# GeoStat-Framework/PyKrige

Hardware: NVIDIA H100
Metric: kriged grid points/sec (N data -> M grid) (higher is better)
Workload: dtype f64

## Files before the change

pykrige_b200/csrc/api.cu:

```cuda
#include <cuda_runtime.h>
#include <string>
#include <vector>
#include <cstring>
#include <cstdio>
#include <cmath>
#include <cstdlib>
#include <algorithm>
#include <thread>
#include <climits>
#include "kernels.h"

#define KB_VERSION 2000
static const int64_t KB_STAGE_PTS = 1 << 20;
#define KB_TILE_COST_32 0.607
#define KB_TILE_COST_16 0.403
static const int64_t KB_STAGE_MIN = 1 << 18;
#define KB_TN_FIELDS 32

struct Src {
    bool grid; int64_t nx, ny, nz;
    const double *a, *b, *c;
    int64_t first, count;
    const double* d_drift; int64_t drift_stride, drift_first;
};

#define KB_GJ_DEFAULT_BLOCKED 1

struct DevBuf {
    void* p = nullptr; size_t cap = 0;
    cudaError_t reserve(size_t bytes) {
        if (bytes <= cap) return cudaSuccess;
        if (p) cudaFree(p);
        p = nullptr; cap = 0;
        cudaError_t e = cudaMalloc(&p, bytes);
        if (e == cudaSuccess) cap = bytes;
        return e;
    }
    void release() { if (p) cudaFree(p); p = nullptr; cap = 0; }
    template <typename T> T* as() const { return reinterpret_cast<T*>(p); }
};

struct kb200_ctx {
    int device = 0;
    cudaStream_t stream = nullptr;
    bool own_stream = false;
    std::string err;

    bool described = false, ready = false, knn_ready = false;
    bool factor_live = false;
    bool inv_live = false;
    int slices = 0;
    int gform = 0;
    int geo = 0;
    int pinv = 0;
    int pinv_sweeps = 0, pinv_rank = 0;
    int dim = 2, dtype = KB200_F64, n = 0, n_pad = 0, ld = 0, n_rl = 0, n_hd = 0, K1 = 1, na = 2, nrb = 0;
    VgParams vg{};
    Aniso an{};
    DriftScale ds{};
    PackMap pm{};
    std::vector<double> hx, hy, hz, hval, hdrift;
    double bb_lo[3] = {0, 0, 0}, bb_hi[3] = {0, 0, 0};
    int nf = 0; int64_t nf_n = 0;
    std::vector<double> hfields;
    int aux_cols = KB_MAXAUX;
    int64_t zstride = 0;
    int pin_blocks = 0;

    DevBuf blob;
    size_t off_consts = 0, off_ax = 0, off_ay = 0, off_az = 0, off_tiles = 0, off_rowscale = 0, blob_bytes = 0;

    DevBuf wC, wW, wT, wF, wRaw, wFlag;
    DevBuf wPart, wAux, wPts, wOut, wAxes, wDrift, wScratch, wFstage;
    int num_sms = 132;
    DeviceDrift dd{};
    DevBuf wWells, wExt;
    int n_dev = 0;
    void* pin[2] = {nullptr, nullptr};
    cudaStream_t copy_stream = nullptr;
    cudaEvent_t evk[2] = {}, evc[2] = {};
    cudaStream_t hi_stream = nullptr;
    std::vector<cudaEvent_t> fev;
    DevBuf kSorted, kCells, kFields;
    DevBuf wVario;
    DevBuf wLoo;
    DevBuf wTab;
    std::vector<double> htab;
    double tab_dmax = 0.0; int tab_n = 0;
    KnnParams kp{};
    int k_ncells = 0;

    cudaEvent_t ev[16] = {};
    double tm[12] = {};
    long long launches = 0, solve_launches = 0;
};

static int fail(kb200_ctx* h, int code, const std::string& msg) {
    if (h) h->err = msg;
    return code;
}
#define CU(h, expr) do { cudaError_t _e = (expr); if (_e != cudaSuccess) { \
    return fail(h, _e == cudaErrorMemoryAllocation ? KB200_ENOMEM : KB200_ECUDA, \
                std::string(#expr) + ": " + cudaGetErrorString(_e)); } } while (0)

static size_t align_up(size_t v, size_t a) { return (v + a - 1) / a * a; }

extern "C" int kb200_version(void) { return KB_VERSION; }

extern "C" int kb200_create(kb200_handle* out, int device) {
    if (!out) return KB200_EBADARG;
    *out = nullptr;
    int cnt = 0;
    cudaError_t e = cudaGetDeviceCount(&cnt);
    if (e != cudaSuccess || cnt == 0) return KB200_ECUDA;
    kb200_ctx* h = new kb200_ctx();
    if (device < 0) { if (cudaGetDevice(&device) != cudaSuccess) device = 0; }
    if (device >= cnt) { delete h; return KB200_EBADARG; }
    h->device = device;
    if (cudaSetDevice(device) != cudaSuccess) { delete h; return KB200_ECUDA; }
    if (cudaStreamCreateWithFlags(&h->stream, cudaStreamNonBlocking) != cudaSuccess) { delete h; return KB200_ECUDA; }
    h->own_stream = true;
    for (auto& ev : h->ev) if (cudaEventCreate(&ev) != cudaSuccess) { delete h; return KB200_ECUDA; }
    if (kbk_factor_init() != cudaSuccess || kbk_solve_init() != cudaSuccess || kbk_solve_tf32_init() != cudaSuccess ||
        kbk_solve_i8_init() != cudaSuccess || kbk_ev_init() != cudaSuccess || kbk_pinv_init() != cudaSuccess) { delete h; return KB200_ECUDA; }
    if (cudaDeviceGetAttribute(&h->num_sms, cudaDevAttrMultiProcessorCount, device) != cudaSuccess || h->num_sms < 1) h->num_sms = 132;
    *out = h;
    return KB200_OK;
}

extern "C" void kb200_destroy(kb200_handle h) {
    if (!h) return;
    cudaSetDevice(h->device);
    cudaStreamSynchronize(h->stream);
    for (DevBuf* b : {&h->blob, &h->wC, &h->wW, &h->wT, &h->wF, &h->wRaw, &h->wFlag, &h->wPart, &h->wAux,
                      &h->wPts, &h->wOut, &h->wAxes, &h->wDrift, &h->wScratch, &h->wFstage, &h->kSorted, &h->kCells, &h->kFields, &h->wVario, &h->wTab,
                      &h->wLoo, &h->wWells, &h->wExt}) b->release();
    for (int i = 0; i < 2; ++i) {
        if (h->pin[i]) cudaFreeHost(h->pin[i]);
        if (h->evk[i]) cudaEventDestroy(h->evk[i]);
        if (h->evc[i]) cudaEventDestroy(h->evc[i]);
    }
    if (h->copy_stream) cudaStreamDestroy(h->copy_stream);
    if (h->hi_stream) cudaStreamDestroy(h->hi_stream);
    for (auto& e : h->fev) cudaEventDestroy(e);
    for (auto& ev : h->ev) if (ev) cudaEventDestroy(ev);
    if (h->own_stream && h->stream) cudaStreamDestroy(h->stream);
    delete h;
}

extern "C" const char* kb200_last_error(kb200_handle h) { return h ? h->err.c_str() : "null handle"; }

extern "C" int kb200_set_stream(kb200_handle h, void* s) {
    if (!h) return KB200_EBADARG;
    if (h->own_stream && h->stream) { cudaStreamSynchronize(h->stream); cudaStreamDestroy(h->stream); }
    h->stream = reinterpret_cast<cudaStream_t>(s);
    h->own_stream = false;
    return KB200_OK;
}

extern "C" int kb200_set_coordinates(kb200_handle h, int coordinates_type) {
    if (!h) return KB200_EBADARG;
    if (coordinates_type != KB200_EUCLIDEAN && coordinates_type != KB200_GEOGRAPHIC)
        return fail(h, KB200_EBADARG, "coordinates_type must be KB200_EUCLIDEAN or KB200_GEOGRAPHIC");
    h->geo = coordinates_type == KB200_GEOGRAPHIC ? 1 : 0;
    h->described = false; h->ready = false; h->knn_ready = false; h->factor_live = false;
    return KB200_OK;
}

extern "C" int kb200_set_pseudo_inverse(kb200_handle h, int enable) {
    if (!h) return KB200_EBADARG;
    h->pinv = enable ? 1 : 0;
    h->described = false; h->ready = false; h->knn_ready = false; h->factor_live = false;
    return KB200_OK;
}

extern "C" int kb200_set_values(kb200_handle h, int n_fields, int64_t n, const double* values) {
    if (!h) return KB200_EBADARG;
    h->described = false; h->ready = false; h->knn_ready = false; h->factor_live = false;
    h->nf = 0; h->nf_n = 0; h->hfields.clear();
    if (n_fields == 0) return KB200_OK;
    if (n_fields < 0 || n_fields > KB200_MAX_FIELDS)
        return fail(h, KB200_EBADARG, "n_fields must be in [0, " + std::to_string(KB200_MAX_FIELDS) + "]");
    if (n < 1 || n > (1LL << 30) || !values) return fail(h, KB200_EBADARG, "values: n >= 1 rows and a non-NULL array");
    const size_t cnt = (size_t)n * n_fields;
    for (size_t i = 0; i < cnt; ++i)
        if (!std::isfinite(values[i]))
            return fail(h, KB200_EBADARG, "values must be finite (field " + std::to_string(i / n) + ", row " +
                        std::to_string(i % n) + ")");
    h->hfields.assign(values, values + cnt);
    h->nf = n_fields; h->nf_n = n;
    return KB200_OK;
}

extern "C" void kb200_reset_counters(kb200_handle h) {
    if (!h) return;
    h->launches = 0; h->solve_launches = 0;
    for (double& t : h->tm) t = 0.0;
}

extern "C" int kb200_last_timings(kb200_handle h, double* ms, int n) {
    if (!h || !ms) return KB200_EBADARG;
    h->tm[10] = (double)h->solve_launches;
    h->tm[11] = (double)h->launches;
    int m = std::min(n, 12);
    for (int i = 0; i < m; ++i) ms[i] = h->tm[i];
    return m;
// ... 348 lines not shown
    CU(h, kbk_dual(h->wW.as<double>(), ld, nn, np, h->n_rl, h->n_hd, nv, ax, ay, az, h->ds, rh, vals,
                   Fz, Hz, Uz, consts, flag, st, &launches));
    if (h->dtype == KB200_F32) {
        CU(h, kbk_pack_tf32(h->wW.as<double>(), ld, nn, np, h->na, Uz, h->pm, blob + h->off_tiles, st));
    } else if (h->slices) {
        const int nrb8 = kbk_i8_nrb(h->slices, nn, h->na);
        std::vector<long long> toff(nrb8 + 1);
        kbk_i8_total_tiles(h->slices, nn, h->na, toff.data());
        long long* d_toff = reinterpret_cast<long long*>(h->wT.as<char>());
        int* d_rowexp = reinterpret_cast<int*>(h->wT.as<char>() + align_up((size_t)(nrb8 + 1) * sizeof(long long), 256));
        CU(h, cudaMemcpyAsync(d_toff, toff.data(), (size_t)(nrb8 + 1) * sizeof(long long), cudaMemcpyHostToDevice, st));
        CU(h, kbk_pack_i8(h->slices, h->wW.as<double>(), ld, nn, np, h->na, Uz, d_rowexp,
                          reinterpret_cast<double*>(blob + h->off_rowscale), d_toff, blob + h->off_tiles, st));
        CU(h, cudaStreamSynchronize(st));
        ++launches;
    } else {
        CU(h, kbk_pack(h->dtype, h->wW.as<double>(), ld, nn, np, h->na, Uz, h->pm, blob + h->off_tiles, st));
    }
    ++launches;
    }
    double hdr[64] = {0};
    hdr[0] = KB_MAGIC; hdr[1] = h->vg.c0; hdr[34] = (double)h->gform;
    for (int c = 0; c <= KB200_MAX_DRIFT; ++c) { hdr[2 + c] = h->ds.shift[c]; hdr[18 + c] = h->ds.scale[c]; }
    CU(h, cudaMemcpyAsync(blob, hdr, sizeof(hdr), cudaMemcpyHostToDevice, st));
    CU(h, cudaEventRecord(h->ev[6], st));
    CU(h, cudaMemcpyAsync(&hflag, flag, sizeof(int), cudaMemcpyDeviceToHost, st));
    CU(h, cudaStreamSynchronize(st));
    h->tm[6] += ev_ms(h->ev[0], h->ev[1]);
    h->tm[0] += t_asm; h->tm[1] += t_chol;
    h->tm[2] += ev_ms(h->ev[4], h->ev[5]);
    h->tm[3] += ev_ms(h->ev[5], h->ev[6]);
    h->launches += launches;
    if (hflag != 0) return fail(h, KB200_ESINGULAR, "drift/unbiasedness block F^T C^-1 F is singular");
    h->ready = true;
    h->factor_live = !h->gform;
    h->inv_live = h->gform != 2;
    return KB200_OK;
}

extern "C" int kb200_set_device_drift(kb200_handle h, int n_wells, const double* wells,
                                      int64_t ext_nx, int64_t ext_ny, const double* ext_x, const double* ext_y,
                                      const double* ext_z) {
    if (!h) return KB200_EBADARG;
    if (n_wells < 0 || n_wells > KB200_MAX_DRIFT || (n_wells > 0 && !wells))
        return fail(h, KB200_EBADARG, "device drift: bad point_log description");
    const bool ext = ext_nx > 0 || ext_ny > 0;
    if (ext && (ext_nx < 1 || ext_ny < 1 || ext_nx > (1 << 30) || ext_ny > (1 << 30) || !ext_x || !ext_y || !ext_z))
        return fail(h, KB200_EBADARG, "device drift: bad external_Z raster description");
    h->described = false; h->ready = false; h->factor_live = false;
    cudaSetDevice(h->device);
    h->dd = DeviceDrift{};
    if (n_wells) {
        CU(h, h->wWells.reserve((size_t)3 * n_wells * 8));
        CU(h, cudaMemcpyAsync(h->wWells.p, wells, (size_t)3 * n_wells * 8, cudaMemcpyHostToDevice, h->stream));
        h->dd.n_wells = n_wells; h->dd.wells = h->wWells.as<double>();
    }
    if (ext) {
        const size_t nx = (size_t)ext_nx, ny = (size_t)ext_ny;
        CU(h, h->wExt.reserve((nx + ny + nx * ny) * 8));
        double* d = h->wExt.as<double>();
        CU(h, cudaMemcpyAsync(d, ext_x, nx * 8, cudaMemcpyHostToDevice, h->stream));
        CU(h, cudaMemcpyAsync(d + nx, ext_y, ny * 8, cudaMemcpyHostToDevice, h->stream));
        CU(h, cudaMemcpyAsync(d + nx + ny, ext_z, nx * ny * 8, cudaMemcpyHostToDevice, h->stream));
        bool sorted = true;
        for (size_t i = 1; i < nx && sorted; ++i) sorted = ext_x[i] >= ext_x[i - 1];
        for (size_t i = 1; i < ny && sorted; ++i) sorted = ext_y[i] >= ext_y[i - 1];
        h->dd.ext = 1; h->dd.ext_nx = (int)ext_nx; h->dd.ext_ny = (int)ext_ny; h->dd.ext_sorted = sorted ? 1 : 0;
        h->dd.ext_x = d; h->dd.ext_y = d + nx; h->dd.ext_z = d + nx + ny;
    }
    CU(h, cudaStreamSynchronize(h->stream));
    return KB200_OK;
}

static int launch_solve(kb200_ctx* h, const Src& s, double* d_z, double* d_ss, int tp) {
    cudaStream_t st = h->stream;
    char* blob = h->blob.as<char>();
    PointSource ps{};
    ps.grid = s.grid ? 1 : 0;
    ps.px = s.a; ps.py = s.b; ps.pz = s.c; ps.gx = s.a; ps.gy = s.b; ps.gz = s.c;
    ps.nx = s.nx; ps.ny = s.ny; ps.nz = s.nz;
    const bool i8 = h->slices != 0;
    const bool f32 = h->dtype == KB200_F32;
    long long ntiles = (s.count + tp - 1) / tp;
    int grid = (int)std::min<long long>(ntiles, h->num_sms);
    CU(h, h->wScratch.reserve(i8 ? kbk_solve_i8_scratch_bytes(h->slices, h->n, grid) : f32 ? kbk_solve_tf32_scratch_bytes(h->n, grid)
                                  : kbk_solve_pt_scratch_doubles(h->n, grid) * sizeof(double)));
    SolvePtParams pp{};
    pp.vg = h->vg; pp.an = h->an; ps.first = s.first; pp.ps = ps;
    pp.n = h->n; pp.na = h->na; pp.nrb = h->nrb; pp.n_rl = h->n_rl; pp.n_hd = h->n_hd;
    pp.ax = reinterpret_cast<double*>(blob + h->off_ax);
    pp.ay = reinterpret_cast<double*>(blob + h->off_ay);
    pp.az = reinterpret_cast<double*>(blob + h->off_az);
    pp.tiles = blob + h->off_tiles; pp.pm = h->pm; pp.ds = h->ds;
    pp.consts = reinterpret_cast<double*>(blob + h->off_consts);
    pp.dd = h->dd; pp.n_dev = h->n_dev;
    pp.drift_pts = s.d_drift; pp.drift_stride = s.drift_stride; pp.drift_first = s.drift_first;
    pp.m = s.count; pp.scratch = h->wScratch.as<double>(); pp.gform = h->gform;
    pp.z_out = d_z; pp.ss_out = d_ss;
    pp.nf = h->nf; pp.zstride = h->zstride;
    if (h->nf) {
        CU(h, h->wFstage.reserve((size_t)grid * h->na * tp * sizeof(double)));
        pp.fstage = h->wFstage.as<double>();
    }
    pp.rowscale = reinterpret_cast<const double*>(blob + h->off_rowscale);
    if (i8) CU(h, kbk_solve_i8(h->slices, h->dim, pp, grid, st));
    else if (f32) CU(h, kbk_solve_tf32(h->dim, pp, grid, st));
    else CU(h, kbk_solve_pt(h->dim, pp, grid, tp, st));
    h->launches += 1; h->solve_launches += 1;
    return KB200_OK;
}

static double tile_cost(int tp) { return tp == 64 ? 1.0 : (tp == 32 ? KB_TILE_COST_32 : KB_TILE_COST_16); }

static int run_solve(kb200_ctx* h, const Src& s, double* d_z, double* d_ss) {
    const bool i8 = h->slices != 0;
    const bool f32 = h->dtype == KB200_F32;
    if (i8 || f32) return launch_solve(h, s, d_z, d_ss, i8 ? kbk_solve_i8_tile_points() : kbk_solve_tf32_tile_points());
    const long long S = h->num_sms;
    const int TW = h->nf ? KB_TN_FIELDS : KB_TN;
    if (const char* e = std::getenv("KB200_TILE")) {
        const int t = std::min(std::atoi(e), TW);
        if (t == 64 || t == 32 || t == 16) return launch_solve(h, s, d_z, d_ss, t);
    }
    const long long nt64 = (s.count + TW - 1) / TW;
    const long long main_pts = std::min<long long>(s.count, (nt64 / S) * S * TW);
    const long long rem = s.count - main_pts;
    if (main_pts > 0) {
        Src m = s; m.count = main_pts;
        int rc = launch_solve(h, m, d_z, d_ss, TW); if (rc) return rc;
    }
    if (rem > 0) {
        int best = TW; double bc = 1e300;
        for (int tp : {64, 32, 16}) {
            if (tp > TW) continue;
            const long long nt = (rem + tp - 1) / tp;
            const double c = (double)((nt + S - 1) / S) * tile_cost(tp);
            if (c < bc * 0.999) { bc = c; best = tp; }
        }
        Src t = s; t.first = s.first + main_pts; t.count = rem; t.drift_first = s.drift_first + main_pts;
        int rc = launch_solve(h, t, d_z + main_pts, d_ss + main_pts, best); if (rc) return rc;
    }
    return KB200_OK;
}

static int run_knn(kb200_ctx* h, int k, const Src& s, double* d_z, double* d_ss, int chol, int loo = 0);

template <class Launch>
static int run_to_host(kb200_ctx* h, int64_t total, double* z_out, double* ss_out, Launch launch) {
    cudaStream_t st = h->stream;
    const int nzb = h->nf ? h->nf : 1;
    h->zstride = total;
    CU(h, h->wOut.reserve((size_t)(nzb + 1) * total * 8));
    double* dz = h->wOut.as<double>();
    double* dss = dz + (size_t)nzb * total;
    CU(h, cudaEventRecord(h->ev[7], st));
    if (total < KB_STAGE_MIN) {
        int rc = launch((int64_t)0, total, dz, dss); if (rc) return rc;
        CU(h, cudaEventRecord(h->ev[8], st));
        CU(h, cudaMemcpyAsync(z_out, dz, (size_t)nzb * total * 8, cudaMemcpyDeviceToHost, st));
        CU(h, cudaMemcpyAsync(ss_out, dss, total * 8, cudaMemcpyDeviceToHost, st));
        CU(h, cudaEventRecord(h->ev[11], st));
        CU(h, cudaStreamSynchronize(st));
        h->tm[7] += ev_ms(h->ev[8], h->ev[11]);
        return KB200_OK;
    }
    if (!h->copy_stream) {
        CU(h, cudaStreamCreateWithFlags(&h->copy_stream, cudaStreamNonBlocking));
        for (int i = 0; i < 2; ++i) {
            CU(h, cudaEventCreateWithFlags(&h->evk[i], cudaEventDisableTiming));
            CU(h, cudaEventCreate(&h->evc[i]));
        }
    }
    if (h->pin_blocks < nzb + 1) {
        for (int i = 0; i < 2; ++i) {
            if (h->pin[i]) { CU(h, cudaFreeHost(h->pin[i])); h->pin[i] = nullptr; }
            CU(h, cudaHostAlloc(&h->pin[i], (size_t)(nzb + 1) * KB_STAGE_PTS * 8, cudaHostAllocDefault));
        }
        h->pin_blocks = nzb + 1;
    }
    const int64_t nch = (total + KB_STAGE_PTS - 1) / KB_STAGE_PTS;
    auto chunk_len = [&](int64_t c) { return std::min<int64_t>(KB_STAGE_PTS, total - c * KB_STAGE_PTS); };
    auto drain = [&](int64_t c) -> int {
        const int b = (int)(c & 1);
        CU(h, cudaEventSynchronize(h->evc[b]));
        const double* p = reinterpret_cast<const double*>(h->pin[b]);
        const int64_t m = chunk_len(c);
        for (int f = 0; f < nzb; ++f)
            std::memcpy(z_out + (size_t)f * total + c * KB_STAGE_PTS, p + (size_t)f * KB_STAGE_PTS, (size_t)m * 8);
        std::memcpy(ss_out + c * KB_STAGE_PTS, p + (size_t)nzb * KB_STAGE_PTS, (size_t)m * 8);
        return KB200_OK;
    };
    for (int64_t c = 0; c < nch; ++c) {
        const int b = (int)(c & 1);
        const int64_t o = c * KB_STAGE_PTS, m = chunk_len(c);
        int rc = launch(o, m, dz + o, dss + o); if (rc) return rc;
        CU(h, cudaEventRecord(h->evk[b], st));
        if (c == nch - 1) CU(h, cudaEventRecord(h->ev[8], st));
        if (c >= 2) { rc = drain(c - 2); if (rc) return rc; }
        double* p = reinterpret_cast<double*>(h->pin[b]);
        CU(h, cudaStreamWaitEvent(h->copy_stream, h->evk[b], 0));
        for (int f = 0; f < nzb; ++f)
// ... 713 lines not shown
```

pykrige_b200/csrc/kernels.h:

```cpp
#pragma once
#include "common.cuh"

struct DriftScale {
    double shift[KB200_MAX_DRIFT + 1];
    double scale[KB200_MAX_DRIFT + 1];
};

struct PackMap {
    int nrb;
    int ktiles[KB_MAXRB];
    long long tile_off[KB_MAXRB];
};

struct DeviceDrift {
    int n_wells;
    int ext;
    int ext_nx, ext_ny;
    int ext_sorted;
    const double* wells;
    const double* ext_x; const double* ext_y; const double* ext_z;
};

struct SolvePtParams {
    VgParams vg;
// ... 74 lines not shown
            double ld = log(sqrt(dx * dx + dy * dy));
            if (isinf(ld)) ld = -100.0;
            f[c] = (-__ldg(P.dd.wells + 3 * w + 2) * ld - P.ds.shift[c]) * P.ds.scale[c];
        }
        if (P.dd.ext) { f[c] = (kb_ext_sample(P.dd, rx, ry) - P.ds.shift[c]) * P.ds.scale[c]; ++c; }
    }
    for (int c = P.n_dev; c < P.n_hd; ++c) {
        double v = P.drift_pts[(size_t)(c - P.n_dev) * P.drift_stride + P.drift_first + pj];
        f[P.n_rl + c] = (v - P.ds.shift[P.n_rl + c]) * P.ds.scale[P.n_rl + c];
    }
    f[K] = 1.0;
    const double zc = (double)aux[K1 * astride];
    const double* Sinv = P.consts;
    const double* phi = P.consts + K1 * K1;
    if (P.gform == 2) {
        double acc = q, zz = zc;
        for (int a = 0; a < K1; ++a) {
            double gf = 0.0;
            for (int b = 0; b < K1; ++b) gf += Sinv[a * K1 + b] * f[b];
            acc += f[a] * (2.0 * (double)aux[a * astride] + gf);
            zz += phi[a] * f[a];
        }
        P.ss_out[pj] = -acc;
        P.z_out[pj] = zz;
        return;
    }
    for (int a = 0; a < K1; ++a) r[a] = (double)aux[a * astride] - f[a];
    if (FIELDS) {
        double rmu = 0.0;
        for (int a = 0; a < K1; ++a) {
            double mu = 0.0;
            for (int b = 0; b < K1; ++b) mu += Sinv[a * K1 + b] * r[b];
            rmu += r[a] * mu;
        }
        P.ss_out[pj] = P.vg.c0 - q + rmu;
        for (int v = 0; v < P.nf; ++v) {
            const double* ph = phi + v * K1;
            double muphi = 0.0;
            for (int a = 0; a < K1; ++a) {
                double mu = 0.0;
                for (int b = 0; b < K1; ++b) mu += Sinv[a * K1 + b] * r[b];
                muphi += mu * ph[a];
            }
            P.z_out[v * P.zstride + pj] = (double)aux[(K1 + v) * astride] - muphi;
        }
        return;
    }
    double rmu = 0.0, muphi = 0.0;
    for (int a = 0; a < K1; ++a) {
        double mu = 0.0;
        for (int b = 0; b < K1; ++b) mu += Sinv[a * K1 + b] * r[b];
        rmu += r[a] * mu;
        muphi += mu * phi[a];
    }
    P.ss_out[pj] = P.vg.c0 - q + rmu;
    P.z_out[pj] = zc - muphi;
}
#endif

cudaError_t kbk_adjust_data(int dim, const Aniso& an, int n, const double* x, const double* y, const double* z,
                            double* ax, double* ay, double* az, cudaStream_t st);
cudaError_t kbk_assemble(int dim, const VgParams& vg, int n, int n_pad, int ld,
                         const double* ax, const double* ay, const double* az, double* C, cudaStream_t st);
cudaError_t kbk_cholesky(double* C, double* W, double* Lstage, int ld, int n_pad, int* flag, double dtol, cudaStream_t st,
                         cudaStream_t hi, cudaEvent_t* ev, int n_ev, int* launches);
cudaError_t kbk_trtri(const double* L, double* W, double* T1, int ld, int n_pad, cudaStream_t st, int* launches);
cudaError_t kbk_dual(const double* W, int ld, int n, int n_pad, int n_rl, int n_hd, int nv,
                     const double* ax, const double* ay, const double* az, const DriftScale& ds,
                     const double* hd, const double* values,
                     double* Fz, double* Hz, double* Uz, double* consts, int* flag, cudaStream_t st, int* launches);
cudaError_t kbk_pack(int dtype, const double* W, int ld, int n, int n_pad, int na, const double* Uz,
                     const PackMap& pm, void* out, cudaStream_t st);

size_t      kbk_general_inverse_workspace_bytes(int n_pad);
cudaError_t kbk_general_inverse(double* C, int ld, int n, int n_pad, void* work, int* flag, double ptol,
                                cudaStream_t st, int* launches, int force_scalar);
cudaError_t kbk_dual_gform(const double* G, int ld, int n, int n_pad, int n_rl, int n_hd, int nv,
                           const double* ax, const double* ay, const double* az, const DriftScale& ds,
                           const double* hd, const double* values,
                           double* Fz, double* Uz, double* consts, int* flag, cudaStream_t st, int* launches);
cudaError_t kbk_pack_gform(const double* G, int ld, int n, int n_pad, int na, const double* Uz,
                           const PackMap& pm, void* out, cudaStream_t st);
cudaError_t kbk_factor_init();
cudaError_t kbk_solve_init();
cudaError_t kbk_solve_pt(int dim, const SolvePtParams& p, int grid, int tile_points , cudaStream_t st);
size_t      kbk_solve_pt_scratch_doubles(int n, int grid);

cudaError_t kbk_solve_tf32_init();
cudaError_t kbk_solve_tf32(int dim, const SolvePtParams& p, int grid, cudaStream_t st);
cudaError_t kbk_pack_tf32(const double* W, int ld, int n, int n_pad, int na, const double* Uz, const PackMap& pm,
                          void* out, cudaStream_t st);
size_t      kbk_solve_tf32_scratch_bytes(int n, int grid);
int         kbk_solve_tf32_tile_points();

bool        kbk_i8_valid_slices(int S);
cudaError_t kbk_solve_i8_init();
cudaError_t kbk_solve_i8(int S, int dim, const SolvePtParams& p, int grid, cudaStream_t st);
cudaError_t kbk_pack_i8(int S, const double* W, int ld, int n, int n_pad, int na, const double* Uz,
                        int* rowexp, double* rowscale, const long long* tile_off_dev, void* out, cudaStream_t st);
int         kbk_i8_nrb(int S, int n, int na);
int         kbk_i8_rows(int S, int n, int na);
long long   kbk_i8_total_tiles(int S, int n, int na, long long* tile_off);
size_t      kbk_i8_tile_bytes(int S);
size_t      kbk_solve_i8_scratch_bytes(int S, int n, int grid);
int         kbk_solve_i8_tile_points();

struct KnnParams {
    VgParams vg;
    Aniso an;
    PointSource ps;
    int dim, n, k;
    const double* ax; const double* ay; const double* az; const double* values;
    const int* sorig;
    int gx, gy, gz;
    int r0;
    double ox, oy, oz, inv_cell, cell;
    const int* cell_start;
    long long m;
    double* z_out; double* ss_out;
    int* flag;
    int nv;
    long long zstride;
};
cudaError_t kbk_knn_build(int dim, int n, const double* ax, const double* ay, const double* az, const double* values,
                          KnnParams& kp, double* sx, double* sy, double* sz, double* sv, int* sorig,
                          int* cell_of, int* cell_start, int* cursor, int ncells, cudaStream_t st, int* launches);
cudaError_t kbk_knn_solve(const KnnParams& p, int chol, cudaStream_t st, int loo = 0);
size_t      kbk_knn_smem_per_warp(int k, int chol, int hasz, int nv);
cudaError_t kbk_knn_sort_fields(int n, int nv, const int* sorig, const double* src, double* dst, cudaStream_t st);

cudaError_t kbk_ev_init();
int         kbk_ev_grid(int n, int num_sms);
size_t      kbk_ev_smem(int nlags, int priv);
int         kbk_ev_priv_max_lags();
cudaError_t kbk_ev_minmax(int dim, int n, const double* x, const double* y, const double* z, int grid,
                          double* bmin, double* bmax, cudaStream_t st);
cudaError_t kbk_ev_bin(int dim, int n, const double* x, const double* y, const double* z, const double* v,
                       int nlags, const double* edges, double inv_dd, int grid, double* part, double* out,
                       cudaStream_t st);
cudaError_t kbk_statistics(int dim, int n, const double* ax, const double* ay, const double* az,
                           const double* L, int ld, const double* u, const double* zeta, int* dup,
                           double* delta, double* sigma, cudaStream_t st);

#define LOO_RC 256
#define LOO_MAXDUP 32
struct LooParams {
    int n, n_pad, ld, K1, nv, gform, nchunks;
    double tol;
    VgParams vg;
    const double* W;
    const double* G;
    const double* part;
    const double* Uz;
    const double* consts;
    const double* Z;
    double* pii; double* alpha;
    double* z_out; double* ss_out;
    int* bad;
};
cudaError_t kbk_loo_colsq(const double* W, int ld, int n, double* part, cudaStream_t st);
cudaError_t kbk_loo_finalize(const LooParams& p, cudaStream_t st);
cudaError_t kbk_loo_pairs(int dim, int n, const double* ax, const double* ay, const double* az, double eps, int* cnt,
                          const int* off, int* pj, double* pd, cudaStream_t st);
cudaError_t kbk_loo_dup(const LooParams& p, int nst, const int* st_list, const int* off, const int* pj, const double* pd,
                        cudaStream_t st);

cudaError_t kbk_build_fz(int n, int n_pad, int n_rl, int n_hd, const double* ax, const double* ay, const double* az,
// ... 8 lines not shown
```

pykrige_b200/csrc/solve.cu:

```cuda
#include "common.cuh"
#include "kernels.h"
#include <cstdlib>

__device__ __forceinline__ uint32_t smem_u32(const void* p) {
    return (uint32_t)__cvta_generic_to_shared(p);
}
__device__ __forceinline__ void mbar_init(uint64_t* bar, int count) {
    asm volatile("mbarrier.init.shared::cta.b64 [%0], %1;\n" :: "r"(smem_u32(bar)), "r"(count));
}
__device__ __forceinline__ void mbar_expect_tx(uint64_t* bar, uint32_t bytes) {
    asm volatile("mbarrier.arrive.expect_tx.shared::cta.b64 _, [%0], %1;\n" :: "r"(smem_u32(bar)), "r"(bytes) : "memory");
}
__device__ __forceinline__ bool mbar_try_wait(uint64_t* bar, uint32_t parity) {
    uint32_t ok;
    asm volatile("{\n\t.reg .pred p;\n\t"
                 "mbarrier.try_wait.parity.shared::cta.b64 p, [%1], %2;\n\t"
                 "selp.u32 %0, 1, 0, p;\n\t}\n"
                 : "=r"(ok) : "r"(smem_u32(bar)), "r"(parity) : "memory");
    return ok != 0;
}
__device__ __forceinline__ void mbar_wait(uint64_t* bar, uint32_t parity) {
    for (uint32_t it = 0; it < (1u << 26); ++it)
        if (mbar_try_wait(bar, parity)) return;
    __trap();
}
__device__ __forceinline__ void bulk_g2s(void* dst, const void* src, uint32_t bytes, uint64_t* bar) {
    asm volatile("cp.async.bulk.shared::cluster.global.mbarrier::complete_tx::bytes [%0], [%1], %2, [%3];\n"
                 :: "r"(smem_u32(dst)), "l"(src), "r"(bytes), "r"(smem_u32(bar)) : "memory");
}

#define PT_STAGES 5
#define PT_THREADS 384
#define PT_CONS0 (PT_THREADS / 32 - 8)
#define PT_STAGE_BYTES ((KB_BM * KB_BK + KB_BK * KB_TN) * 8)

__device__ __forceinline__ void mbar_arrive(uint64_t* bar) {
    asm volatile("mbarrier.arrive.shared::cta.b64 _, [%0];\n" :: "r"(smem_u32(bar)) : "memory");
}

template <int C>
__device__ __forceinline__ void pt_reduce_scatter_step(double* v, int lane, int mask) {
    if constexpr (C >= 2) {
        const bool up = (lane & mask) != 0;
#pragma unroll
        for (int h = 0; h < C / 2; ++h) {
            const double send = up ? v[h] : v[h + C / 2];
            const double keep = up ? v[h + C / 2] : v[h];
            v[h] = keep + __shfl_xor_sync(0xffffffffu, send, mask);
        }
    } else {
        v[0] += __shfl_xor_sync(0xffffffffu, v[0], mask);
    }
}
template <int CNT>
__device__ __forceinline__ void pt_reduce_scatter(double* v, int lane) {
    pt_reduce_scatter_step<CNT>(v, lane, 16);
    pt_reduce_scatter_step<(CNT >= 2 ? CNT / 2 : 1)>(v, lane, 8);
    pt_reduce_scatter_step<(CNT >= 4 ? CNT / 4 : 1)>(v, lane, 4);
}
template <int CNT>
__device__ __forceinline__ int pt_reduce_scatter_index(int i, int lane) {
    int o = i, c = CNT;
    for (int mask = 16; mask >= 4; mask >>= 1) {
        if (c >= 2) { c /= 2; if (lane & mask) o += c; }
        else if (lane & mask) return -1;
    }
    return o;
}

template <int DIM, int MODEL, int NT, bool FIELDS>
__global__ void __launch_bounds__(PT_THREADS, 1) solve_kernel_pt(const __grid_constant__ SolvePtParams P) {
    constexpr int TN = NT * 8;
    extern __shared__ __align__(128) unsigned char smem_raw[];
    double* Ts = reinterpret_cast<double*>(smem_raw);
    double* Bs = Ts + PT_STAGES * KB_BM * KB_BK;
    double* qred = Bs + PT_STAGES * KB_BK * TN;
    double* auxs = qred + 8 * TN;
    uint64_t* full = reinterpret_cast<uint64_t*>(auxs + KB_MAXAUX * TN);
    uint64_t* empty = full + PT_STAGES;

    const int tid = threadIdx.x, lane = tid & 31, warp = tid >> 5;
    const int nk = (P.n + KB_BK - 1) / KB_BK;
    double* scratch = P.scratch + (size_t)blockIdx.x * nk * (KB_BK * TN);
    const double* gt = reinterpret_cast<const double*>(P.tiles);
    const long long ntiles = (P.m + TN - 1) / TN;

    if (tid == 0) {
        for (int s = 0; s < PT_STAGES; ++s) { mbar_init(&full[s], 1); mbar_init(&empty[s], 8); }
        asm volatile("fence.mbarrier_init.release.cluster;\n" ::: "memory");
        asm volatile("fence.proxy.async.shared::cta;\n" ::: "memory");
    }
    __syncthreads();

    const uint32_t stages_per_tile = (uint32_t)(P.pm.tile_off[P.nrb - 1] + P.pm.ktiles[P.nrb - 1]);
    const int cw = warp - PT_CONS0;

    for (uint32_t it = 0; blockIdx.x + (long long)it * gridDim.x < ntiles; ++it) {
        const long long tile = blockIdx.x + (long long)it * gridDim.x;
        const uint32_t git = it * stages_per_tile;
        {
            const int pl = tid % TN;
            const int ks = tid / TN;
            const long long pj = tile * TN + pl;
            const bool pvalid = pj < P.m;
            double px = 0.0, py = 0.0, pz = 0.0;
            if (pvalid) kb_load_point<DIM>(P.ps, P.an, pj, px, py, pz);
            for (int t = ks; t < nk; t += PT_THREADS / TN) {
                double* bt = scratch + (size_t)t * (KB_BK * TN);
#pragma unroll
                for (int k4 = 0; k4 < 4; ++k4) {
                    double v[4];
#pragma unroll
                    for (int kk = 0; kk < 4; ++kk) {
                        const int k = t * KB_BK + k4 * 4 + kk;
                        double val = 0.0;
                        if (pvalid && k < P.n) {
                            double d = kb_dist<DIM>(__ldg(P.ax + k), __ldg(P.ay + k), KB_HASZ(DIM) ? __ldg(P.az + k) : 0.0,
                                                    px, py, pz);
                            val = kb_cov_rhs<MODEL>(P.vg, d);
                        }
                        v[kk] = val;
                    }
                    double2* dst = reinterpret_cast<double2*>(bt + (k4 * NT + (pl >> 3)) * 32 + (pl & 7) * 4);
                    dst[0] = make_double2(v[0], v[1]);
                    dst[1] = make_double2(v[2], v[3]);
                }
            }
            __threadfence();
            asm volatile("fence.proxy.async.global;\n" ::: "memory");
        }
        __syncthreads();

        if (warp == 0) {
            if (lane == 0) {
                uint32_t g = git;
                const uint64_t pol_w = kb_policy_evict_last(), pol_c = kb_policy_evict_first();
                long long tau = 0;
                for (int I = 0; I < P.nrb; ++I) {
                    const int kt = P.pm.ktiles[I];
                    for (int t = 0; t < kt; ++t, ++tau, ++g) {
                        const int s = g % PT_STAGES;
                        mbar_wait(&empty[s], (uint32_t)(((g / PT_STAGES) & 1) ^ 1));
                        mbar_expect_tx(&full[s], (KB_BM * KB_BK + KB_BK * TN) * 8);
                        kb_bulk_g2s_hint(Ts + (size_t)s * KB_BM * KB_BK, gt + (size_t)tau * (KB_BM * KB_BK),
                                         KB_BM * KB_BK * 8, &full[s], pol_w);
                        kb_bulk_g2s_hint(Bs + (size_t)s * KB_BK * TN, scratch + (size_t)t * (KB_BK * TN),
                                         KB_BK * TN * 8, &full[s], pol_c);
                    }
                }
            }
        } else if (warp >= PT_CONS0) {
            uint32_t g = git;
            constexpr int QV = NT >= 4 ? NT / 4 : 1;
            double* qrow = qred + cw * TN;
#pragma unroll
            for (int v = 0; v < QV; ++v) {
                const int o = pt_reduce_scatter_index<2 * NT>(v, lane);
                if (o >= 0) qrow[(o >> 1) * 8 + 2 * (lane & 3) + (o & 1)] = 0.0;
            }
            const int mtl[2] = {cw, 15 - cw};
            for (int I = 0; I < P.nrb; ++I) {
                const uint32_t gend = g + (uint32_t)P.pm.ktiles[I];
                uint32_t glim[2];
#pragma unroll
                for (int q = 0; q < 2; ++q) {
                    const int r0 = I * KB_BM + mtl[q] * 16;
                    if (r0 + 15 >= P.n && r0 < P.n + P.na) glim[q] = gend;
                    else if (r0 >= P.n + P.na) glim[q] = g;
                    else glim[q] = g + (uint32_t)(r0 / KB_BK + 1);
                }
                double acc[2][NT][4];
#pragma unroll
                for (int a = 0; a < 2; ++a)
#pragma unroll
                    for (int b = 0; b < NT; ++b)
#pragma unroll
                        for (int i = 0; i < 4; ++i) acc[a][b][i] = 0.0;
                for (; g < gend; ++g) {
                    const int s = g % PT_STAGES;
                    mbar_wait(&full[s], (uint32_t)((g / PT_STAGES) & 1));
                    const bool on0 = g < glim[0], on1 = g < glim[1];
                    if (on0 || on1) {
                        const double2* ts = reinterpret_cast<const double2*>(Ts + (size_t)s * KB_BM * KB_BK);
                        const double* bs = Bs + (size_t)s * KB_BK * TN;
#pragma unroll
                        for (int k4 = 0; k4 < 4; ++k4) {
                            double fa[2][2];
#pragma unroll
                            for (int q = 0; q < 2; ++q) {
                                const double2 v = ts[(mtl[q] * 4 + k4) * 32 + lane];
                                fa[q][0] = v.x; fa[q][1] = v.y;
                            }
#pragma unroll
                            for (int nt = 0; nt < NT; ++nt) {
                                const double fb = bs[(k4 * NT + nt) * 32 + lane];
                                if (on0) kb_dmma_16x8x4(acc[0][nt], fa[0], fb);
                                if (on1) kb_dmma_16x8x4(acc[1][nt], fa[1], fb);
                            }
                        }
                    }
                    __syncwarp();
                    if (lane == 0) mbar_arrive(&empty[s]);
                }
#pragma unroll
                for (int q = 0; q < 2; ++q)
#pragma unroll
                    for (int h = 0; h < 2; ++h) {
                        const int r = I * KB_BM + mtl[q] * 16 + 8 * h + (lane >> 2);
                        if (r < P.n) {
                            if (!P.gform) {
#pragma unroll
                                for (int nt = 0; nt < NT; ++nt)
#pragma unroll
                                    for (int i = 0; i < 2; ++i) acc[q][nt][2 * h + i] *= acc[q][nt][2 * h + i];
                            } else {
                                const double* bt = P.scratch + ((size_t)blockIdx.x * nk + (r >> 4)) * (KB_BK * TN) +
                                                   ((r & 15) >> 2) * (NT * 32) + (r & 3);
#pragma unroll
                                for (int nt = 0; nt < NT; ++nt)
#pragma unroll
                                    for (int i = 0; i < 2; ++i) {
                                        const int c = nt * 8 + 2 * (lane & 3) + i;
                                        acc[q][nt][2 * h + i] *= bt[(c >> 3) * 32 + (c & 7) * 4];
                                    }
                            }
                        } else {
                            if (r < P.n + P.na) {
                                double* ao = (FIELDS ? P.fstage + (int)(blockIdx.x * P.na * TN) : auxs) + (r - P.n) * TN +
                                             2 * (lane & 3);
#pragma unroll
                                for (int nt = 0; nt < NT; ++nt) {
                                    ao[nt * 8] = acc[q][nt][2 * h];
                                    ao[nt * 8 + 1] = acc[q][nt][2 * h + 1];
                                }
                            }
#pragma unroll
                            for (int nt = 0; nt < NT; ++nt) { acc[q][nt][2 * h] = 0.0; acc[q][nt][2 * h + 1] = 0.0; }
                        }
                    }
                double part[2 * NT];
#pragma unroll
                for (int nt = 0; nt < NT; ++nt)
#pragma unroll
                    for (int i = 0; i < 2; ++i)
                        part[2 * nt + i] = ((acc[0][nt][i] + acc[0][nt][2 + i]) + acc[1][nt][i]) + acc[1][nt][2 + i];
                pt_reduce_scatter<2 * NT>(part, lane);
#pragma unroll
                for (int v = 0; v < QV; ++v) {
                    const int o = pt_reduce_scatter_index<2 * NT>(v, lane);
                    if (o >= 0) qrow[(o >> 1) * 8 + 2 * (lane & 3) + (o & 1)] += part[v];
                }
            }
        }
        __syncthreads();

        if (tid < TN) {
            const long long pj = tile * TN + tid;
            if (pj < P.m) {
                double q = 0.0;
#pragma unroll
                for (int w = 0; w < 8; ++w) q += qred[w * TN + tid];
                if constexpr (FIELDS)
                    kb_finalize_point<DIM, double, true>(P, pj, q, P.fstage + (int)(blockIdx.x * P.na * TN) + tid, TN);
                else
                    kb_finalize_point<DIM, double>(P, pj, q, auxs + tid, TN);
            }
        }
        __syncthreads();
    }
}

static size_t solve_smem_pt() {
    return (size_t)PT_STAGES * (KB_BM * KB_BK + KB_BK * KB_TN) * sizeof(double) + 8 * KB_TN * sizeof(double) +
           KB_MAXAUX * KB_TN * sizeof(double) + 2 * PT_STAGES * sizeof(uint64_t) + 64;
}
size_t kbk_solve_pt_scratch_doubles(int n, int grid) {
    return (size_t)grid * ((n + KB_BK - 1) / KB_BK) * (KB_BK * KB_TN);
}


template <int DIM, int MODEL, bool FIELDS>
static cudaError_t solve_set_attr_f() {
    constexpr int NT8 = FIELDS ? 4 : 8;
    KB_CUDA_OK(cudaFuncSetAttribute(solve_kernel_pt<DIM, MODEL, NT8, FIELDS>, cudaFuncAttributeMaxDynamicSharedMemorySize,
                                    (int)solve_smem_pt()));
    KB_CUDA_OK(cudaFuncSetAttribute(solve_kernel_pt<DIM, MODEL, 4, FIELDS>, cudaFuncAttributeMaxDynamicSharedMemorySize,
                                    (int)solve_smem_pt()));
    return cudaFuncSetAttribute(solve_kernel_pt<DIM, MODEL, 2, FIELDS>, cudaFuncAttributeMaxDynamicSharedMemorySize,
                                (int)solve_smem_pt());
}
template <int DIM, int MODEL>
static cudaError_t solve_set_attr() {
    KB_CUDA_OK((solve_set_attr_f<DIM, MODEL, false>()));
    return solve_set_attr_f<DIM, MODEL, true>();
}

cudaError_t kbk_solve_init() {
#define KB_ATTR(M) KB_CUDA_OK((solve_set_attr<2, M>())); KB_CUDA_OK((solve_set_attr<3, M>())); KB_CUDA_OK((solve_set_attr<KB_GEO, M>()));
    KB_ATTR(KB200_VG_LINEAR) KB_ATTR(KB200_VG_POWER) KB_ATTR(KB200_VG_GAUSSIAN)
    KB_ATTR(KB200_VG_EXPONENTIAL) KB_ATTR(KB200_VG_SPHERICAL) KB_ATTR(KB200_VG_HOLE_EFFECT) KB_ATTR(KB200_VG_TABLE)
#undef KB_ATTR
    return cudaSuccess;
}

template <int DIM, bool FIELDS>
static cudaError_t solve_pt_dim(const SolvePtParams& p, int grid, int tile_points, cudaStream_t st) {
    size_t sm = solve_smem_pt();
    constexpr int NT8 = FIELDS ? 4 : 8;
    if (FIELDS && tile_points == 64) return cudaErrorInvalidValue;
    switch (p.vg.model) {
#define KB_CASE(M) case M: if (tile_points == 16) solve_kernel_pt<DIM, M, 2, FIELDS><<<grid, PT_THREADS, sm, st>>>(p); \
                           else if (tile_points == 32) solve_kernel_pt<DIM, M, 4, FIELDS><<<grid, PT_THREADS, sm, st>>>(p); \
                           else solve_kernel_pt<DIM, M, NT8, FIELDS><<<grid, PT_THREADS, sm, st>>>(p); break;
        KB_CASE(KB200_VG_LINEAR) KB_CASE(KB200_VG_POWER) KB_CASE(KB200_VG_GAUSSIAN)
        KB_CASE(KB200_VG_EXPONENTIAL) KB_CASE(KB200_VG_SPHERICAL) KB_CASE(KB200_VG_HOLE_EFFECT) KB_CASE(KB200_VG_TABLE)
#undef KB_CASE
        default: return cudaErrorInvalidValue;
    }
    return cudaGetLastError();
}

cudaError_t kbk_solve_pt(int dim, const SolvePtParams& p, int grid, int tile_points, cudaStream_t st) {
    if (tile_points != 64 && tile_points != 32 && tile_points != 16) return cudaErrorInvalidValue;
    if (p.nf) {
        if (dim == KB_GEO) return solve_pt_dim<KB_GEO, true>(p, grid, tile_points, st);
        return dim == 2 ? solve_pt_dim<2, true>(p, grid, tile_points, st) : solve_pt_dim<3, true>(p, grid, tile_points, st);
    }
    if (dim == KB_GEO) return solve_pt_dim<KB_GEO, false>(p, grid, tile_points, st);
    return dim == 2 ? solve_pt_dim<2, false>(p, grid, tile_points, st) : solve_pt_dim<3, false>(p, grid, tile_points, st);
}
```

Before: 1.795 million.

## Pair solve CTAs in 2-CTA clusters and multicast shared weight tiles

The f64 solve kernel now launches as 2-CTA thread block clusters. Each CTA loads half of every shared KB_BM×KB_BK weight tile and multicasts it to both CTAs, so per-CTA L2/global traffic for that operand is halved. The empty barriers now count arrivals from both CTAs, using remote mbarrier arrives, and the grid is sized from cluster occupancy and rounded to even tile counts. The tile-cost heuristics are also retuned. The cost is tighter cross-CTA coupling: the paired CTAs stall on each other's consumers, and extra cluster syncs are added.

```diff
diff --git a/pykrige_b200/csrc/api.cu b/pykrige_b200/csrc/api.cu
--- a/pykrige_b200/csrc/api.cu
+++ b/pykrige_b200/csrc/api.cu
@@ -12,8 +12,8 @@
 
 #define KB_VERSION 2000
 static const int64_t KB_STAGE_PTS = 1 << 20;
-#define KB_TILE_COST_32 0.607
-#define KB_TILE_COST_16 0.403
+#define KB_TILE_COST_32 0.569
+#define KB_TILE_COST_16 0.330
 static const int64_t KB_STAGE_MIN = 1 << 18;
 #define KB_TN_FIELDS 32
 
@@ -73,6 +73,7 @@
     DevBuf wC, wW, wT, wF, wRaw, wFlag;
     DevBuf wPart, wAux, wPts, wOut, wAxes, wDrift, wScratch, wFstage;
     int num_sms = 132;
+    int solve_ctas = 0;
     DeviceDrift dd{};
     DevBuf wWells, wExt;
     int n_dev = 0;
@@ -121,7 +122,7 @@
     if (cudaStreamCreateWithFlags(&h->stream, cudaStreamNonBlocking) != cudaSuccess) { delete h; return KB200_ECUDA; }
     h->own_stream = true;
     for (auto& ev : h->ev) if (cudaEventCreate(&ev) != cudaSuccess) { delete h; return KB200_ECUDA; }
-    if (kbk_factor_init() != cudaSuccess || kbk_solve_init() != cudaSuccess || kbk_solve_tf32_init() != cudaSuccess ||
+    if (kbk_factor_init() != cudaSuccess || kbk_solve_init(&h->solve_ctas) != cudaSuccess || kbk_solve_tf32_init() != cudaSuccess ||
         kbk_solve_i8_init() != cudaSuccess || kbk_ev_init() != cudaSuccess || kbk_pinv_init() != cudaSuccess) { delete h; return KB200_ECUDA; }
     if (cudaDeviceGetAttribute(&h->num_sms, cudaDevAttrMultiProcessorCount, device) != cudaSuccess || h->num_sms < 1) h->num_sms = 132;
     *out = h;
@@ -636,7 +637,8 @@
     const bool i8 = h->slices != 0;
     const bool f32 = h->dtype == KB200_F32;
     long long ntiles = (s.count + tp - 1) / tp;
-    int grid = (int)std::min<long long>(ntiles, h->num_sms);
+    int grid = (i8 || f32) ? (int)std::min<long long>(ntiles, h->num_sms)
+                           : (int)std::min<long long>(2 * ((ntiles + 1) / 2), h->solve_ctas);
     CU(h, h->wScratch.reserve(i8 ? kbk_solve_i8_scratch_bytes(h->slices, h->n, grid) : f32 ? kbk_solve_tf32_scratch_bytes(h->n, grid)
                                   : kbk_solve_pt_scratch_doubles(h->n, grid) * sizeof(double)));
     SolvePtParams pp{};
@@ -670,7 +672,7 @@
     const bool i8 = h->slices != 0;
     const bool f32 = h->dtype == KB200_F32;
     if (i8 || f32) return launch_solve(h, s, d_z, d_ss, i8 ? kbk_solve_i8_tile_points() : kbk_solve_tf32_tile_points());
-    const long long S = h->num_sms;
+    const long long S = h->solve_ctas;
     const int TW = h->nf ? KB_TN_FIELDS : KB_TN;
     if (const char* e = std::getenv("KB200_TILE")) {
         const int t = std::min(std::atoi(e), TW);
diff --git a/pykrige_b200/csrc/kernels.h b/pykrige_b200/csrc/kernels.h
--- a/pykrige_b200/csrc/kernels.h
+++ b/pykrige_b200/csrc/kernels.h
@@ -180,7 +180,7 @@
 cudaError_t kbk_pack_gform(const double* G, int ld, int n, int n_pad, int na, const double* Uz,
                            const PackMap& pm, void* out, cudaStream_t st);
 cudaError_t kbk_factor_init();
-cudaError_t kbk_solve_init();
+cudaError_t kbk_solve_init(int* max_ctas);
 cudaError_t kbk_solve_pt(int dim, const SolvePtParams& p, int grid, int tile_points , cudaStream_t st);
 size_t      kbk_solve_pt_scratch_doubles(int n, int grid);
 
diff --git a/pykrige_b200/csrc/solve.cu b/pykrige_b200/csrc/solve.cu
--- a/pykrige_b200/csrc/solve.cu
+++ b/pykrige_b200/csrc/solve.cu
@@ -24,6 +24,25 @@
         if (mbar_try_wait(bar, parity)) return;
     __trap();
 }
+__device__ __forceinline__ void mbar_arrive_remote(uint64_t* bar, uint32_t rank) {
+    uint32_t rbar;
+    asm volatile("mapa.shared::cluster.u32 %0, %1, %2;\n" : "=r"(rbar) : "r"(smem_u32(bar)), "r"(rank));
+    asm volatile("mbarrier.arrive.shared::cluster.b64 _, [%0];\n" :: "r"(rbar) : "memory");
+}
+__device__ __forceinline__ void bulk_g2s_pair(void* dst, const void* src, uint32_t bytes, uint64_t* bar, uint64_t policy) {
+    asm volatile("cp.async.bulk.shared::cluster.global.mbarrier::complete_tx::bytes.multicast::cluster.L2::cache_hint"
+                 " [%0], [%1], %2, [%3], %4, %5;\n"
+                 :: "r"(smem_u32(dst)), "l"(src), "r"(bytes), "r"(smem_u32(bar)), "h"((uint16_t)0x3), "l"(policy)
+                 : "memory");
+}
+__device__ __forceinline__ void cluster_sync() {
+    asm volatile("barrier.cluster.arrive.release.aligned;\n\tbarrier.cluster.wait.acquire.aligned;\n" ::: "memory");
+}
+__device__ __forceinline__ uint32_t cluster_ctarank() {
+    uint32_t r;
+    asm volatile("mov.u32 %0, %%cluster_ctarank;\n" : "=r"(r));
+    return r;
+}
 __device__ __forceinline__ void bulk_g2s(void* dst, const void* src, uint32_t bytes, uint64_t* bar) {
     asm volatile("cp.async.bulk.shared::cluster.global.mbarrier::complete_tx::bytes [%0], [%1], %2, [%3];\n"
                  :: "r"(smem_u32(dst)), "l"(src), "r"(bytes), "r"(smem_u32(bar)) : "memory");
@@ -69,7 +88,7 @@
 }
 
 template <int DIM, int MODEL, int NT, bool FIELDS>
-__global__ void __launch_bounds__(PT_THREADS, 1) solve_kernel_pt(const __grid_constant__ SolvePtParams P) {
+__global__ void __cluster_dims__(2, 1, 1) __launch_bounds__(PT_THREADS, 1) solve_kernel_pt(const __grid_constant__ SolvePtParams P) {
     constexpr int TN = NT * 8;
     extern __shared__ __align__(128) unsigned char smem_raw[];
     double* Ts = reinterpret_cast<double*>(smem_raw);
@@ -84,19 +103,20 @@
     double* scratch = P.scratch + (size_t)blockIdx.x * nk * (KB_BK * TN);
     const double* gt = reinterpret_cast<const double*>(P.tiles);
     const long long ntiles = (P.m + TN - 1) / TN;
+    const uint32_t rank = cluster_ctarank(), pair = blockIdx.x >> 1, npairs = gridDim.x >> 1;
 
     if (tid == 0) {
-        for (int s = 0; s < PT_STAGES; ++s) { mbar_init(&full[s], 1); mbar_init(&empty[s], 8); }
+        for (int s = 0; s < PT_STAGES; ++s) { mbar_init(&full[s], 1); mbar_init(&empty[s], 16); }
         asm volatile("fence.mbarrier_init.release.cluster;\n" ::: "memory");
         asm volatile("fence.proxy.async.shared::cta;\n" ::: "memory");
     }
-    __syncthreads();
+    cluster_sync();
 
     const uint32_t stages_per_tile = (uint32_t)(P.pm.tile_off[P.nrb - 1] + P.pm.ktiles[P.nrb - 1]);
     const int cw = warp - PT_CONS0;
 
-    for (uint32_t it = 0; blockIdx.x + (long long)it * gridDim.x < ntiles; ++it) {
-        const long long tile = blockIdx.x + (long long)it * gridDim.x;
+    for (uint32_t it = 0; 2 * (pair + (long long)it * npairs) < ntiles; ++it) {
+        const long long tile = 2 * (pair + (long long)it * npairs) + rank;
         const uint32_t git = it * stages_per_tile;
         {
             const int pl = tid % TN;
@@ -142,8 +162,9 @@
                         const int s = g % PT_STAGES;
                         mbar_wait(&empty[s], (uint32_t)(((g / PT_STAGES) & 1) ^ 1));
                         mbar_expect_tx(&full[s], (KB_BM * KB_BK + KB_BK * TN) * 8);
-                        kb_bulk_g2s_hint(Ts + (size_t)s * KB_BM * KB_BK, gt + (size_t)tau * (KB_BM * KB_BK),
-                                         KB_BM * KB_BK * 8, &full[s], pol_w);
+                        constexpr int HALF = KB_BM * KB_BK / 2;
+                        bulk_g2s_pair(Ts + (size_t)s * KB_BM * KB_BK + rank * HALF,
+                                      gt + (size_t)tau * (KB_BM * KB_BK) + rank * HALF, HALF * 8, &full[s], pol_w);
                         kb_bulk_g2s_hint(Bs + (size_t)s * KB_BK * TN, scratch + (size_t)t * (KB_BK * TN),
                                          KB_BK * TN * 8, &full[s], pol_c);
                     }
@@ -200,7 +221,7 @@
                         }
                     }
                     __syncwarp();
-                    if (lane == 0) mbar_arrive(&empty[s]);
+                    if (lane == 0) { mbar_arrive(&empty[s]); mbar_arrive_remote(&empty[s], rank ^ 1); }
                 }
 #pragma unroll
                 for (int q = 0; q < 2; ++q)
@@ -268,6 +289,7 @@
         }
         __syncthreads();
     }
+    cluster_sync();
 }
 
 static size_t solve_smem_pt() {
@@ -295,11 +317,17 @@
     return solve_set_attr_f<DIM, MODEL, true>();
 }
 
-cudaError_t kbk_solve_init() {
+cudaError_t kbk_solve_init(int* max_ctas) {
 #define KB_ATTR(M) KB_CUDA_OK((solve_set_attr<2, M>())); KB_CUDA_OK((solve_set_attr<3, M>())); KB_CUDA_OK((solve_set_attr<KB_GEO, M>()));
     KB_ATTR(KB200_VG_LINEAR) KB_ATTR(KB200_VG_POWER) KB_ATTR(KB200_VG_GAUSSIAN)
     KB_ATTR(KB200_VG_EXPONENTIAL) KB_ATTR(KB200_VG_SPHERICAL) KB_ATTR(KB200_VG_HOLE_EFFECT) KB_ATTR(KB200_VG_TABLE)
 #undef KB_ATTR
+    cudaLaunchConfig_t cfg{};
+    cfg.gridDim = dim3(2); cfg.blockDim = dim3(PT_THREADS); cfg.dynamicSmemBytes = solve_smem_pt();
+    int pairs = 0;
+    KB_CUDA_OK(cudaOccupancyMaxActiveClusters(&pairs, solve_kernel_pt<2, KB200_VG_EXPONENTIAL, 8, false>, &cfg));
+    if (pairs < 1) return cudaErrorInvalidConfiguration;
+    *max_ctas = 2 * pairs;
     return cudaSuccess;
 }
 
@@ -322,6 +350,7 @@
 
 cudaError_t kbk_solve_pt(int dim, const SolvePtParams& p, int grid, int tile_points, cudaStream_t st) {
     if (tile_points != 64 && tile_points != 32 && tile_points != 16) return cudaErrorInvalidValue;
+    if (grid < 2 || (grid & 1)) return cudaErrorInvalidValue;
     if (p.nf) {
         if (dim == KB_GEO) return solve_pt_dim<KB_GEO, true>(p, grid, tile_points, st);
         return dim == 2 ? solve_pt_dim<2, true>(p, grid, tile_points, st) : solve_pt_dim<3, true>(p, grid, tile_points, st);
```

Result: faster. 1.817 million, median of 6 (+1.2%).
